# liortalker/MindTheEdge

Hardware: AMD Instinct MI355X
Metric: training images/sec, PackNet-SAN+edge-loss 384x1280 bf16 (higher is better)
Workload: dtype bf16; 1 GPU; T8: PackNet-SAN + silog + 4-scale depth-edge loss training step, 384x1280, 8 frames/GPU, dropout 0.5, flip 0.5; global_batch=8, height=384, width=1280, parallelism=single GPU

## Files before the change

include/mte_kernels.h:

```cpp
#ifndef MTE_KERNELS_H
#define MTE_KERNELS_H

#ifdef __cplusplus
extern "C" {
#endif

typedef struct ihipStream_t* mte_stream_t;

#define MTE_OK 0
#define MTE_ERR_ARG (-1)
#define MTE_ERR_LAUNCH (-2)
#define MTE_ERR_UNSUPPORTED (-3)
#define MTE_DT_BF16 0
#define MTE_DT_F32 1

#define MTE_CONV_ACCUMULATE 1
#define MTE_CONV_SOLO 2
int mte_conv2d_igemm(const void* x, long ldx, const void* wpack, const float* bias, void* y, long ldy, int out_f32,
                     int B, int H, int W, int Cin_p, int N, int KH, int KW, int dtype,
                     float* workspace, long workspace_elems, int accumulate, mte_stream_t stream);
int mte_conv2d_igemm_unshuffle(const void* x, long ldx, const void* wpack, void* y, long ldy,
                               int B, int H, int W, int Cin_p, int N, int KH, int KW, int dtype, int accumulate, mte_stream_t stream);
#define MTE_OPT_GN_PREZEROED 0
#define MTE_OPT_LOSS_PREZEROED 1
// ... 49 lines not shown
                   int B, int HW, int C, float eps, int dtype, mte_stream_t stream);
int mte_gn_tail_fwd(const void* y1, long ld1, const double* stats1, const float* gamma1, const float* beta1,
                    const void* y2, long ld2, const float* scale2, void* t, long ldt, double* stats_t,
                    const float* gamma_t, const float* beta_t, void* z, long ldz,
                    int B, int HW, int C, float eps, int dtype, mte_stream_t stream);

int mte_pack3d_fwd(const void* x, long ldx, const float* w3, const float* b3, void* out, long ldo,
                   int B, int H, int W, int C, int dtype, mte_stream_t stream);
int mte_pack3d_bwd_data(const void* dout, long ldo, const float* w3, void* dx, long lddx,
                        int B, int H, int W, int C, int dtype, mte_stream_t stream);
int mte_pack3d_bwd_weight(const void* x, long ldx, const void* dout, long ldo, float* dwb,
                          int B, int H, int W, int C, int dtype, mte_stream_t stream);
int mte_unpack3d_fwd(const void* x, long ldx, const float* w3, const float* b3, void* out, long ldo,
                     int B, int H, int W, int C, int dtype, mte_stream_t stream);
int mte_unpack3d_bwd_data(const void* dout, long ldo, const float* w3, void* dx, long lddx,
                          int B, int H, int W, int C, int dtype, mte_stream_t stream);
int mte_unpack3d_bwd_weight(const void* x, long ldx, const void* dout, long ldo, float* dwb,
                            int B, int H, int W, int C, int dtype, mte_stream_t stream);

int mte_fold_pack_weights(const float* W, const float* K3, const float* b, const float* b3, float* Wf, float* bf,
                          int Co, int D, int k, mte_stream_t stream);
int mte_unfold_pack_wgrad(const float* dWf, const float* dbf, const float* W, const float* K3, const float* b3,
                          float* dW, float* dk3b, int Co, int D, int k, int accumulate, mte_stream_t stream);
int mte_pixel_shuffle(const void* src, long lds_, void* dst, long ldd, int B, int H, int W, int C, int dir, int dtype, mte_stream_t stream);
int mte_copy_rect(const void* src, long lds_, int Hs, int Ws, int sy, int sx, void* dst, long ldd, int Hd, int Wd, int dy, int dx,
                  int B, int h, int w, int C, int mode, int dtype, mte_stream_t stream);
typedef struct { const void* src; long lds_; int Hs, Ws, sy, sx; void* dst; long ldd; int Hd, Wd, dy, dx, h, w, mode; } mte_rect_op;
int mte_copy_rects(const void* ops, int n, int B, int C, int dtype, mte_stream_t stream);

int mte_invdepth_fwd(const void* x, long ldx, const float* w, const float* bias, float* out,
                     int B, int H, int W, int C, float min_depth, int dtype, mte_stream_t stream);
int mte_invdepth_bwd_data(const float* w, const float* inv_out, const float* dout, float* dlogit,
                          void* dx, long lddx, int B, int H, int W, int C, float min_depth, int dtype, mte_stream_t stream);
long mte_invdepth_bwd_weight_workspace_elems(int C);
int mte_invdepth_bwd_weight(const void* x, long ldx, const float* dlogit, float* dwb, float* records,
                            int B, int H, int W, int C, int dtype, mte_stream_t stream);

int mte_rank1_conv_fwd(const float* inv, const float* w, long w_stride, void* y, long ldy, int B, int h, int wl, int N, int dtype, mte_stream_t stream);
int mte_rank1_conv_bwd_data(const void* dy, long lddy, const float* w, long w_stride, float* dinv, int B, int h, int wl, int N, int accumulate, int dtype,
                            mte_stream_t stream);
int mte_upsample2_f32(const float* inv, float* out, int B, int h, int wl, mte_stream_t stream);
int mte_conv2d_patch_fwd_rank1_ok(const float* bias, long ldx, int B, int H, int W, int Cin_p, int N);
int mte_conv2d_patch_fwd_rank1(const void* x, long ldx, const void* wpatch, const float* bias, void* y, long ldy, int B, int H, int W, int Cin_p, int N,
                               const float* inv, const float* w1, long w1_stride, mte_stream_t stream);
int mte_conv2d_patch_fwd_plus1x1(const void* x, long ldx, const void* wpatch, const float* bias, void* y, long ldy, int B, int H, int W, int Cin_p, int N,
                                 const void* x2, long ldx2, const void* wpatch2, int C2, mte_stream_t stream);
long mte_rank1_conv_bwd_records_elems(int N);
int mte_rank1_conv_bwd_weight(const void* dy, long lddy, const float* inv, float* dw, long dw_stride, float* records,
                              int B, int h, int wl, int N, int dtype, mte_stream_t stream);
int mte_nchw_to_nhwc(const float* src, void* dst, long ldd, int B, int C, int H, int W, int Cp, int flip_w, int dtype, mte_stream_t stream);
int mte_upsample_inv_fwd(const float* inv, void* dst, long ldd, int B, int h, int w, int dtype, mte_stream_t stream);
int mte_upsample_inv_bwd(const void* dsrc, long lds_, float* dinv, int B, int h, int w, int accumulate, int dtype, mte_stream_t stream);
int mte_copy_channels(const void* src, long lds_, void* dst, long ldd, long npix, int C, int dtype, mte_stream_t stream);
int mte_split_record(const float* src, float* dst0, int n0, float* dst1, int n1, mte_stream_t stream);
int mte_add_channels(const void* a, long lda, const void* b, long ldb, void* out, long ldo, long npix, int C, int dtype, mte_stream_t stream);

typedef struct { const float* pred; const float* edge; const float* normal; const float* mask; float* gmap; float* dpred; int H; int W; } mte_edge_scale;
long mte_edge_loss_work_elems(const void* scales, int nscales, int B);
int mte_edge_loss_multi_fwd(const void* scales, int nscales, int B, int from_inv, int is_grad, int is_sigmoid, float thresh,
                            float weight, float pos_to_neg, const float* gt_depth, double* work, float* losses, float* coef,
                            float* silog_loss, float* silog_aux, mte_stream_t stream);
int mte_edge_loss_multi_bwd(const void* scales, int nscales, int B, int from_inv, int is_grad, int is_sigmoid, float thresh,
                            const float* coef, const float* gout, const float* gt_depth, const float* silog_aux, const float* silog_gout,
                            mte_stream_t stream);
long mte_edge_loss_sums_elems(int B, int H, int W);
int mte_edge_loss_fwd(const float* pred, const float* edge, const float* normal, const float* mask, double* sums, float* gmap,
                      int B, int H, int W, int from_inv, int is_grad, int is_sigmoid, float thresh, mte_stream_t stream);
int mte_edge_loss_finalize(const double* sums, int B, long numel, float weight, float pos_to_neg, int has_mask,
                           float out_scale, float* loss_acc, float* loss_this, float* coef, mte_stream_t stream);
int mte_edge_loss_bwd(const float* pred, const float* edge, const float* normal, const float* mask, const float* coef, const float* gout,
                      float* dpred, int B, int H, int W, int from_inv, int is_grad, int is_sigmoid, float thresh, mte_stream_t stream);

long mte_edge_loss_kind_work_elems(int B, int H, int W);
// ... 105 lines not shown
```

mindtheedge_amd/csrc/heads_misc.hip:

```cpp
#include "common.hpp"
#include <atomic>

int tap_wgrad_mfma_launch(const bf16_t* x, long ldx, const float* m, float* rec, long rec_stride, int B, int H, int W, int C, int sgn, int up2, int has_db,
                          int max_wgs, int* groups, hipStream_t st);
namespace {

template <typename T> __device__ __forceinline__ void ld8(const T* p, float* v);
template <> __device__ __forceinline__ void ld8<bf16_t>(const bf16_t* p, float* v) { unpack16<bf16_t>(*(const u32x4_t*)p, v); }
template <> __device__ __forceinline__ void ld8<float>(const float* p, float* v) {
    unpack16<float>(*(const u32x4_t*)p, v); unpack16<float>(*(const u32x4_t*)(p + 4), v + 4);
}
template <typename T> __device__ __forceinline__ void st8(T* p, const float* v);
template <> __device__ __forceinline__ void st8<bf16_t>(bf16_t* p, const float* v) { *(u32x4_t*)p = pack16<bf16_t>(v); }
template <> __device__ __forceinline__ void st8<float>(float* p, const float* v) {
    *(u32x4_t*)p = pack16<float>(v); *(u32x4_t*)(p + 4) = pack16<float>(v + 4);
}

struct HeadArgs {
    const void* x; long ldx;
    const float* w; const float* bias;
    float* out;
    const float* dlogit;
    void* dx; long lddx;
    float* dw;
// ... 153 lines not shown
            for (int s = 0; s < CS; ++s) in[kx][s] = nxt[kx][s];
        if constexpr (PF) { if (r < y1) load_row(r + 1); }
        f32x4_t d = {0.f, 0.f, 0.f, 0.f};
#pragma unroll
        for (int kx = 0; kx < 3; ++kx)
#pragma unroll
            for (int s = 0; s < CS; ++s) {
                d = __builtin_amdgcn_mfma_f32_16x16x32_bf16(__builtin_bit_cast(bf16x8_t, wh[kx][s]), __builtin_bit_cast(bf16x8_t, in[kx][s]), d, 0, 0, 0);
                d = __builtin_amdgcn_mfma_f32_16x16x32_bf16(__builtin_bit_cast(bf16x8_t, wl[kx][s]), __builtin_bit_cast(bf16x8_t, in[kx][s]), d, 0, 0, 0);
            }
        const float done = o_prev + d[2];
        if (kb == 0 && r - 1 >= y0 && r - 1 < y1 && x < a.W) out[(long)(r - 1) * a.W + x] = a.inv_min_depth / (1.f + __expf(-(done + bias)));
        o_prev = o_cur + d[1];
        o_cur = d[0];
    }
}

__global__ void invdepth_dlogit_kernel(const float* __restrict__ dout, const float* __restrict__ inv, float* __restrict__ dl, long n, float s) {
    for (long i = blockIdx.x * (long)blockDim.x + threadIdx.x; i < n; i += (long)gridDim.x * blockDim.x) {
        const float v = inv[i];
        dl[i] = dout[i] * v * (1.f - v / s);
    }
}

struct DlRow { float v[3]; bool ok; };
#define HEAD_LOAD_DL(Y, D)                                                                        \
    {                                                                                             \
        (D).ok = (unsigned)(Y) < (unsigned)a.H;                                                   \
        const long row_ = (long)min(max((Y), 0), a.H - 1) * a.W;                                  \
        _Pragma("unroll") for (int cx = 0; cx < 3; ++cx) (D).v[cx] = dl[row_ + xc[cx]];           \
    }
#define HEAD_DL(D, CX) (((D).ok && xok[CX]) ? (D).v[CX] : 0.f)

template <typename T>
__global__ __launch_bounds__(256) void invdepth_bwd_data_kernel(HeadArgs a) {
    HEAD_MAP();
    float wr[9][8];
#pragma unroll
    for (int t = 0; t < 9; ++t)
#pragma unroll
        for (int i = 0; i < 8; ++i) wr[t][i] = a.w[(c0 + i) * 9 + t];
#pragma unroll 1
    for (int strip = s_first; strip < s_last; ++strip) {
        HEAD_STRIP();
        const float* dl = a.dlogit + (long)b * a.H * a.W;
        T* dx = (T*)a.dx + (long)b * a.H * a.W * a.lddx + c0;
        DlRow d[4];
        HEAD_LOAD_DL(y0 - 1, d[0]) HEAD_LOAD_DL(y0, d[1]) HEAD_LOAD_DL(y0 + 1, d[2])
#define HEAD_BD_STEP(K, R0, R1, R2, R3)                                                           \
    {                                                                                             \
        const int yy = y + K;                                                                     \
        HEAD_LOAD_DL(yy + 2, d[R3])                                                               \
        float dxv[8];                                                                             \
        _Pragma("unroll") for (int i = 0; i < 8; ++i) dxv[i] = 0.f;                               \
        _Pragma("unroll") for (int ty = 0; ty < 3; ++ty)                                          \
            _Pragma("unroll") for (int tx = 0; tx < 3; ++tx) {                                    \
                const float g = ty == 0 ? HEAD_DL(d[R2], 2 - tx) : (ty == 1 ? HEAD_DL(d[R1], 2 - tx) : HEAD_DL(d[R0], 2 - tx)); \
                _Pragma("unroll") for (int i = 0; i < 8; ++i) dxv[i] = fmaf(g, wr[ty * 3 + tx][i], dxv[i]); \
            }                                                                                     \
        if (xin && yy < y1) st8<T>(dx + ((long)yy * a.W + x) * a.lddx, dxv);                      \
    }
        for (int y = y0; y < y1; y += 4) {
            HEAD_BD_STEP(0, 0, 1, 2, 3) HEAD_BD_STEP(1, 1, 2, 3, 0) HEAD_BD_STEP(2, 2, 3, 0, 1) HEAD_BD_STEP(3, 3, 0, 1, 2)
        }
#undef HEAD_BD_STEP
    }
}

template <typename T>
__global__ __launch_bounds__(256) void invdepth_bwd_weight_kernel(HeadArgs a) {
    extern __shared__ float sdw[];
    for (int i = threadIdx.x; i < a.C * 9 + 1; i += 256) sdw[i] = 0.f;
    __syncthreads();
    HEAD_MAP();
    float gw[9][8];
#pragma unroll
    for (int t = 0; t < 9; ++t)
#pragma unroll
        for (int i = 0; i < 8; ++i) gw[t][i] = 0.f;
    float gb = 0.f;
#pragma unroll 1
    for (int strip = s_first; strip < s_last; ++strip) {
        HEAD_STRIP();
        const float* dl = a.dlogit + (long)b * a.H * a.W;
        const T* img = (const T*)a.x + (long)b * a.H * a.W * a.ldx + c0;
        DlRow d[5];
        Ch8<T> xr[4];
        bool xrok[4];
#define HEAD_LOAD_X(Y, S) { xrok[S] = xin && (Y) < y1; xr[S].load(img + ((long)min((Y), a.H - 1) * a.W + xc[1]) * a.ldx); }
        HEAD_LOAD_DL(y0 - 1, d[0]) HEAD_LOAD_DL(y0, d[1]) HEAD_LOAD_DL(y0 + 1, d[2]) HEAD_LOAD_DL(y0 + 2, d[3])
        HEAD_LOAD_X(y0, 0) HEAD_LOAD_X(y0 + 1, 1) HEAD_LOAD_X(y0 + 2, 2)
#define HEAD_BW_STEP(K, R0, R1, R2, R4, X0, X3)                                                   \
// ... 185 lines not shown
                const bool kk = ok && Yok[r];
                win[r][k] = u32x4_t{kk ? v[0] : 0u, kk ? v[1] : 0u, kk ? v[2] : 0u, kk ? v[3] : 0u};
            }
        };
#pragma unroll
        for (int k = 0; k < 4; ++k) load_col(2 * x0 - 1 + k, k);
        const int x1 = min(x0 + SEG, wl);
        for (int x = x0; x < x1; ++x) {
            float acc = 0.f;
            const int woff = cc * P;
#pragma unroll
            for (int r = 0; r < 4; ++r)
#pragma unroll
                for (int k = 0; k < 4; ++k) {
                    float g[P];
                    unpack16<T>(win[r][k], g);
                    const float* wr = wc + (r * 4 + k) * N + woff;
#pragma unroll
                    for (int e = 0; e < P; ++e) acc = fmaf(g[e], wr[e], acc);
                }
            for (int off = 1; off < cpr; off <<= 1) acc += __shfl_xor(acc, off, 64);
            const long pq = ((long)b * h + yl) * wl + x;
            if (live && cc == 0) dinv[pq] = accumulate ? dinv[pq] + acc : acc;
            if (x + 1 < x1) {
#pragma unroll
                for (int r = 0; r < 4; ++r) { win[r][0] = win[r][2]; win[r][1] = win[r][3]; }
                load_col(2 * x + 3, 2);
                load_col(2 * x + 4, 3);
            }
        }
    }
}

template <typename T>
__global__ __launch_bounds__(256) void rank1_conv_bwd_weight_kernel(const T* __restrict__ dy, long lddy, const float* __restrict__ inv, float* __restrict__ records,
                                                                    int B, int h, int wl, int N) {
    extern __shared__ __attribute__((aligned(16))) float sred[];
    constexpr int P = Elem<T>::PER16, SEG = 16;
    const int cpr = N / P, W = 2 * wl, nseg = (wl + SEG - 1) / SEG;
    const long items = (long)B * h * nseg * cpr;
    float dacc[9][P];
#pragma unroll
    for (int tp = 0; tp < 9; ++tp)
#pragma unroll
        for (int e = 0; e < P; ++e) dacc[tp][e] = 0.f;
    const int cc = threadIdx.x % cpr;
    for (long it = blockIdx.x * (long)blockDim.x + threadIdx.x; it < items; it += (long)gridDim.x * blockDim.x) {
        long t = it / cpr;
        const int x0 = (int)(t % nseg) * SEG; t /= nseg;
        const int yl = (int)(t % h); const int b = (int)(t / h);
        const T* base = dy + (((long)b * 2 * h + 2 * yl) * W) * lddy + cc * P;
        const float* ir[3]; bool iok[3];
#pragma unroll
        for (int r = 0; r < 3; ++r) { const int yy = yl - 1 + r; iok[r] = (unsigned)yy < (unsigned)h; ir[r] = inv + ((long)b * h + min(max(yy, 0), h - 1)) * wl; }
        float uw[3][3];
#pragma unroll
        for (int k = 0; k < 3; ++k) {
            const int xx = x0 - 1 + k; const bool ok = (unsigned)xx < (unsigned)wl; const int xc = min(max(xx, 0), wl - 1);
#pragma unroll
            for (int r = 0; r < 3; ++r) uw[r][k] = (ok && iok[r]) ? ir[r][xc] : 0.f;
        }
        const int x1 = min(x0 + SEG, wl);
        for (int x = x0; x < x1; ++x) {
            u32x4_t raw[4];
#pragma unroll
            for (int q = 0; q < 4; ++q) raw[q] = *(const u32x4_t*)(base + ((long)(q >> 1) * W + 2 * x + (q & 1)) * lddy);
// ... 136 lines not shown
    float src = scale * ((float)dst + 0.5f) - 0.5f;
    if (src < 0.f) src = 0.f;
    i0 = (int)src; if (i0 > in - 1) i0 = in - 1;
    i1 = i0 < in - 1 ? i0 + 1 : i0;
    l1 = src - (float)i0;
}
__global__ void resize_bilinear_kernel(const float* __restrict__ x, float* __restrict__ y, float* __restrict__ dx, const float* __restrict__ dy,
                                       int B, int h, int w, int H, int W) {
    const float sh = (float)h / (float)H, sw = (float)w / (float)W;
    const long n = (long)B * H * W;
    for (long i = blockIdx.x * (long)blockDim.x + threadIdx.x; i < n; i += (long)gridDim.x * blockDim.x) {
        const int X = (int)(i % W), Y = (int)((i / W) % H), b = (int)(i / ((long)W * H));
        int y0, y1, x0, x1; float ly, lx;
        bilin_src(Y, h, sh, y0, y1, ly); bilin_src(X, w, sw, x0, x1, lx);
        const long base = (long)b * h * w;
        const float w00 = (1.f - ly) * (1.f - lx), w01 = (1.f - ly) * lx, w10 = ly * (1.f - lx), w11 = ly * lx;
        if (y) {
            y[i] = w00 * x[base + (long)y0 * w + x0] + w01 * x[base + (long)y0 * w + x1] + w10 * x[base + (long)y1 * w + x0] + w11 * x[base + (long)y1 * w + x1];
        } else {
            const float g = dy[i];
            atomicAdd(dx + base + (long)y0 * w + x0, w00 * g); atomicAdd(dx + base + (long)y0 * w + x1, w01 * g);
            atomicAdd(dx + base + (long)y1 * w + x0, w10 * g); atomicAdd(dx + base + (long)y1 * w + x1, w11 * g);
        }
    }
}

inline int stream_grid(long n, int per = 256) { long g = (n + per - 1) / per; return (int)(g > 8192 ? 8192 : (g < 1 ? 1 : g)); }
int g_head_mfma = 1;
inline bool head_ok(int C) { const int cb = C >> 3; return C % 8 == 0 && cb >= 1 && cb <= 64 && (cb & (cb - 1)) == 0; }
inline long head_strips(int B, int H, int W, int C) {
    const int pxw = 256 / (C >> 3);
    return (long)((W + pxw - 1) / pxw) * ((H + HEAD_ROWS - 1) / HEAD_ROWS) * B;
}
template <typename F> int head_resident(F f, size_t lds, std::atomic<int>* cache) {
    int v = cache->load(std::memory_order_relaxed);
    if (v == 0) {
        int per_cu = 0, dev = 0, cus = 256;
        if (hipOccupancyMaxActiveBlocksPerMultiprocessor(&per_cu, f, 256, lds) != hipSuccess || per_cu < 1) per_cu = 2;
        hipDeviceProp_t prop;
        if (hipGetDevice(&dev) == hipSuccess && hipGetDeviceProperties(&prop, dev) == hipSuccess && prop.multiProcessorCount > 0) cus = prop.multiProcessorCount;
        v = per_cu * cus;
        cache->store(v, std::memory_order_relaxed);
    }
    return v;
}
inline long head_record_stride(int C) { return ((long)C * 9 + 1 + 3) / 4 * 4; }
constexpr int HEAD_WGRAD_MAX_BLOCKS = 1024;

}

#ifdef MTE_DEV
extern "C" int mtei_set_head_mfma(int v) { g_head_mfma = v; return MTE_OK; }
#endif

extern "C" {

int mte_invdepth_fwd(const void* x, long ldx, const float* w, const float* bias, float* out,
                     int B, int H, int W, int C, float min_depth, int dtype, hipStream_t stream) {
    (void)hipGetLastError();
    if (!x || !w || !bias || !out || !head_ok(C)) return MTE_ERR_ARG;
    HeadArgs a{}; a.x = x; a.ldx = ldx; a.w = w; a.bias = bias; a.out = out; a.B = B; a.H = H; a.W = W; a.C = C;
    a.inv_min_depth = 1.f / min_depth; a.npix = (long)B * H * W;
    if (dtype == MTE_DT_BF16 && g_head_mfma && C % 32 == 0 && C <= ((g_head_mfma & 2) ? 256 : 128) && ldx % 8 == 0) {
        int rows = C >= 128 ? 16 : 32;
        bool pf = C >= 64;
        if (g_head_mfma != 1) {
            pf = (g_head_mfma & 4) != 0;
            if (g_head_mfma >> 8) rows = g_head_mfma >> 8;
        }
        const long g2 = (long)((W + 63) / 64) * ((H + rows - 1) / rows) * B;
        if (g2 <= 0x7fffffffL) {
#define MTE_HEAD_LAUNCH(CS_)                                                                                                              \
            if (pf) hipLaunchKernelGGL((invdepth_fwd_mfma_kernel<CS_, true>), dim3((unsigned)g2), dim3(256), 0, stream, a, rows);       \
            else hipLaunchKernelGGL((invdepth_fwd_mfma_kernel<CS_, false>), dim3((unsigned)g2), dim3(256), 0, stream, a, rows);         \
            return mte_check_launch();
            switch (C / 32) {
                case 1: { MTE_HEAD_LAUNCH(1) }
                case 2: { MTE_HEAD_LAUNCH(2) }
                case 4: { MTE_HEAD_LAUNCH(4) }
                case 8: { MTE_HEAD_LAUNCH(8) }
            }
#undef MTE_HEAD_LAUNCH
        }
    }
    const long grid = head_strips(B, H, W, C);
    if (grid > 0x7fffffffL) return MTE_ERR_UNSUPPORTED;
    if (dtype == MTE_DT_BF16) hipLaunchKernelGGL(invdepth_fwd_kernel<bf16_t>, dim3((unsigned)grid), dim3(256), 0, stream, a);
    else hipLaunchKernelGGL(invdepth_fwd_kernel<float>, dim3((unsigned)grid), dim3(256), 0, stream, a);
    return mte_check_launch();
}

int mte_invdepth_bwd_data(const float* w, const float* inv_out, const float* dout, float* dlogit,
                          void* dx, long lddx, int B, int H, int W, int C, float min_depth, int dtype, hipStream_t stream) {
    (void)hipGetLastError();
    if (!w || !inv_out || !dout || !dlogit || !dx || !head_ok(C)) return MTE_ERR_ARG;
    const long npix = (long)B * H * W;
    hipLaunchKernelGGL(invdepth_dlogit_kernel, dim3(stream_grid(npix)), dim3(256), 0, stream, dout, inv_out, dlogit, npix, 1.f / min_depth);
    HeadArgs a{}; a.w = w; a.dlogit = dlogit; a.dx = dx; a.lddx = lddx; a.B = B; a.H = H; a.W = W; a.C = C; a.npix = npix;
    const long grid = head_strips(B, H, W, C);
    if (grid > 0x7fffffffL) return MTE_ERR_UNSUPPORTED;
    if (dtype == MTE_DT_BF16) hipLaunchKernelGGL(invdepth_bwd_data_kernel<bf16_t>, dim3((unsigned)grid), dim3(256), 0, stream, a);
    else hipLaunchKernelGGL(invdepth_bwd_data_kernel<float>, dim3((unsigned)grid), dim3(256), 0, stream, a);
    return mte_check_launch();
}

long mte_invdepth_bwd_weight_workspace_elems(int C) { return head_ok(C) ? HEAD_WGRAD_MAX_BLOCKS * head_record_stride(C) : 0; }

int mte_invdepth_bwd_weight(const void* x, long ldx, const float* dlogit, float* dwb, float* records,
                            int B, int H, int W, int C, int dtype, hipStream_t stream) {
    (void)hipGetLastError();
    if (!x || !dlogit || !dwb || !records || !head_ok(C)) return MTE_ERR_ARG;
    const long npix = (long)B * H * W;
    HeadArgs a{}; a.x = x; a.ldx = ldx; a.dlogit = dlogit; a.dw = records; a.rec_stride = head_record_stride(C);
    a.B = B; a.H = H; a.W = W; a.C = C; a.npix = npix;
    const int n = C * 9 + 1;
    if (dtype == MTE_DT_BF16) {
        int groups = 0;
        const int rc = tap_wgrad_mfma_launch((const bf16_t*)x, ldx, dlogit, records, a.rec_stride, B, H, W, C, -1, 0, 1, HEAD_WGRAD_MAX_BLOCKS, &groups, stream);
        if (rc == MTE_OK) {
            hipLaunchKernelGGL(invdepth_reduce_kernel, dim3((n + 63) / 64), dim3(1024), 0, stream, records, a.rec_stride, groups, n, dwb);
            return mte_check_launch();
        }
        if (rc != MTE_ERR_UNSUPPORTED) return rc;
    }
    const size_t lds = sizeof(float) * (C * 9 + 4);
    long g = head_strips(B, H, W, C);
    static std::atomic<int> res_b[64], res_f[64];
    const int ci = (C >> 3) & 63;
    const long res = dtype == MTE_DT_BF16 ? head_resident(invdepth_bwd_weight_kernel<bf16_t>, lds, &res_b[ci]) : head_resident(invdepth_bwd_weight_kernel<float>, lds, &res_f[ci]);
    if (g > res) g = res;
    if (g > HEAD_WGRAD_MAX_BLOCKS) g = HEAD_WGRAD_MAX_BLOCKS;
    if (dtype == MTE_DT_BF16) hipLaunchKernelGGL(invdepth_bwd_weight_kernel<bf16_t>, dim3((unsigned)g), dim3(256), lds, stream, a);
    else hipLaunchKernelGGL(invdepth_bwd_weight_kernel<float>, dim3((unsigned)g), dim3(256), lds, stream, a);
    hipLaunchKernelGGL(invdepth_reduce_kernel, dim3((n + 63) / 64), dim3(1024), 0, stream, records, a.rec_stride, (int)g, n, dwb);
    return mte_check_launch();
}
// ... 14 lines not shown
    if (dtype == MTE_DT_BF16) hipLaunchKernelGGL(upsample_inv_kernel<bf16_t>, dim3(grid), dim3(256), 0, stream, inv, (bf16_t*)dst, ldd, B, h, w);
    else hipLaunchKernelGGL(upsample_inv_kernel<float>, dim3(grid), dim3(256), 0, stream, inv, (float*)dst, ldd, B, h, w);
    return mte_check_launch();
}
int mte_upsample_inv_bwd(const void* dsrc, long lds_, float* dinv, int B, int h, int w, int accumulate, int dtype, hipStream_t stream) {
    (void)hipGetLastError();
    if (!dsrc || !dinv) return MTE_ERR_ARG;
    const int grid = stream_grid((long)B * h * w);
    if (dtype == MTE_DT_BF16) hipLaunchKernelGGL(upsample_inv_bwd_kernel<bf16_t>, dim3(grid), dim3(256), 0, stream, (const bf16_t*)dsrc, lds_, dinv, B, h, w, accumulate);
    else hipLaunchKernelGGL(upsample_inv_bwd_kernel<float>, dim3(grid), dim3(256), 0, stream, (const float*)dsrc, lds_, dinv, B, h, w, accumulate);
    return mte_check_launch();
}

int mte_rank1_conv_fwd(const float* inv, const float* w, long w_stride, void* y, long ldy, int B, int h, int wl, int N, int dtype, hipStream_t stream) {
    (void)hipGetLastError();
    if (!inv || !w || !y || N % 32 != 0 || N > 256 || B < 1 || h < 1 || wl < 1) return MTE_ERR_ARG;
    const int per16 = dtype == MTE_DT_BF16 ? 8 : 4;
    const int grid = stream_grid((long)B * 2 * h * ((2 * wl + 63) / 64) * (N / per16));
    if (dtype == MTE_DT_BF16) hipLaunchKernelGGL(rank1_conv_fwd_kernel<bf16_t>, dim3(grid), dim3(256), 0, stream, inv, w, w_stride, (bf16_t*)y, ldy, B, h, wl, N);
    else hipLaunchKernelGGL(rank1_conv_fwd_kernel<float>, dim3(grid), dim3(256), 0, stream, inv, w, w_stride, (float*)y, ldy, B, h, wl, N);
    return mte_check_launch();
}
int mte_rank1_conv_bwd_data(const void* dy, long lddy, const float* w, long w_stride, float* dinv, int B, int h, int wl, int N, int accumulate, int dtype,
                            hipStream_t stream) {
    (void)hipGetLastError();
    if (!dy || !w || !dinv || (N != 32 && N != 64 && N != 128) || B < 1 || h < 1 || wl < 1) return MTE_ERR_ARG;
    const int per16 = dtype == MTE_DT_BF16 ? 8 : 4;
    const int grid = stream_grid((long)B * h * ((wl + 15) / 16) * (N / per16));
    const size_t lds = sizeof(float) * 25 * N;
    if (dtype == MTE_DT_BF16) hipLaunchKernelGGL(rank1_conv_bwd_data_kernel<bf16_t>, dim3(grid), dim3(256), lds, stream, (const bf16_t*)dy, lddy, w, w_stride, dinv, B, h, wl, N, accumulate);
    else hipLaunchKernelGGL(rank1_conv_bwd_data_kernel<float>, dim3(grid), dim3(256), lds, stream, (const float*)dy, lddy, w, w_stride, dinv, B, h, wl, N, accumulate);
    return mte_check_launch();
}
constexpr int RANK1_BWD_WGS = 1024;
long mte_rank1_conv_bwd_records_elems(int N) { return (long)RANK1_BWD_WGS * N * 9; }
int mte_rank1_conv_bwd_weight(const void* dy, long lddy, const float* inv, float* dw, long dw_stride, float* records,
                              int B, int h, int wl, int N, int dtype, hipStream_t stream) {
    (void)hipGetLastError();
    if (!dy || !inv || !dw || !records || (N != 32 && N != 64 && N != 128) || B < 1 || h < 1 || wl < 1) return MTE_ERR_ARG;
    if (dtype == MTE_DT_BF16) {
        int groups = 0;
        const int rc = tap_wgrad_mfma_launch((const bf16_t*)dy, lddy, inv, records, (long)N * 9, B, 2 * h, 2 * wl, N, +1, 1, 0, RANK1_BWD_WGS, &groups, stream);
        if (rc == MTE_OK) {
            hipLaunchKernelGGL(rank1_wgrad_reduce_kernel, dim3((N * 9 + 3) / 4), dim3(256), 0, stream, records, groups, N, dw, dw_stride);
            return mte_check_launch();
        }
        if (rc != MTE_ERR_UNSUPPORTED) return rc;
    }
    const int per16 = dtype == MTE_DT_BF16 ? 8 : 4;
    const long items = (long)B * h * ((wl + 15) / 16) * (N / per16);
    long g = (items + 255) / 256; if (g > RANK1_BWD_WGS) g = RANK1_BWD_WGS; if (g < 1) g = 1;
    const size_t lds = sizeof(float) * 4 * N * 9;
    if (dtype == MTE_DT_BF16) hipLaunchKernelGGL(rank1_conv_bwd_weight_kernel<bf16_t>, dim3((unsigned)g), dim3(256), lds, stream, (const bf16_t*)dy, lddy, inv, records, B, h, wl, N);
    else hipLaunchKernelGGL(rank1_conv_bwd_weight_kernel<float>, dim3((unsigned)g), dim3(256), lds, stream, (const float*)dy, lddy, inv, records, B, h, wl, N);
    hipLaunchKernelGGL(rank1_wgrad_reduce_kernel, dim3((N * 9 + 3) / 4), dim3(256), 0, stream, records, (int)g, N, dw, dw_stride);
    return mte_check_launch();
}
int mte_upsample2_f32(const float* inv, float* out, int B, int h, int wl, hipStream_t stream) {
    (void)hipGetLastError();
    if (!inv || !out || B < 1 || h < 1 || wl < 1) return MTE_ERR_ARG;
    hipLaunchKernelGGL(upsample2_f32_kernel, dim3(stream_grid((long)B * 4 * h * wl)), dim3(256), 0, stream, inv, out, B, h, wl);
    return mte_check_launch();
}

int mte_copy_channels(const void* src, long lds_, void* dst, long ldd, long npix, int C, int dtype, hipStream_t stream) {
    (void)hipGetLastError();
// ... 61 lines not shown
```

mindtheedge_amd/kernels.py:

```python
import ctypes
import itertools
import math
import os
import weakref

import torch

from ._lib import lib, MteError

DT_BF16, DT_F32 = 0, 1
_state = {"compute_dtype": torch.bfloat16, "weights_epoch": 0}


def set_compute_dtype(dtype):
    dtype = {"bf16": torch.bfloat16, "fp32": torch.float32, "f32": torch.float32}.get(dtype, dtype)
    assert dtype in (torch.bfloat16, torch.float32)
    _state["compute_dtype"] = dtype


def compute_dtype():
    return _state["compute_dtype"]


def bump_weights_epoch():
# ... 870 lines not shown
        yp, ldy = _pl(y)
        w1 = w.detach().data_ptr() + 4 * cm * 9
        xp, ldx = _pl(x)
        if (_cfg["fuse_inv_term"] and pack is not None and _patch_ok(W, Cp, cout, kh, kw, x.dtype)
                and lib.mte_conv2d_patch_fwd_rank1_ok(_ptr(b), ldx, B, H, W, Cp, cout) == 1):
            lib.mte_conv2d_patch_fwd_rank1(xp, ldx, pack.get_patch(wm, 'f').data_ptr(), _ptr(b), yp, ldy, B, H, W, Cp, cout,
                                           invc.data_ptr(), w1, cin * 9, _stream())
        else:
            lib.mte_rank1_conv_fwd(invc.data_ptr(), w1, cin * 9, yp, ldy, B, H // 2, W // 2, cout, _dt(y), _stream())
            conv_forward(x, wf, b, cout, kh, kw, out=y, pack=pack, w=wm, accumulate=True)
        z, stats = _gn_forward(y, None, None, gamma, beta, GN_EPS, out=None if out is None else alias_of(out))
        ctx.save_for_backward(x, invc, w, wm, y, stats, gamma, beta)
        ctx.pack = pack
        ctx.bias = b
        return z

    @staticmethod
    def backward(ctx, dz):
        x, invc, w, wm, y, stats, gamma, beta = ctx.saved_tensors
        b = ctx.bias
        cout, cin, kh, kw = w.shape
        cm = cin - 1
        B, Cp, H, W = x.shape
        gg, sg = _grad_dst(gamma, zero=True)
        gb, sb = _grad_dst(beta, zero=True)
        gbias, sbias = _grad_dst(b, zero=True)
        gw, sw = _grad_dst(w)
        dy, _, dgamma, dbeta, db = _gn_backward(dz, y, None, None, stats, gamma, beta, GN_EPS, False, want_dbias=True,
                                                dgamma=gg, dbeta=gb, dbias=gbias)
        dyp, lddy = _pl(dy)

        dinv = torch.empty((B, 1, H // 2, W // 2), dtype=torch.float32, device=x.device)
        wl = w.detach()
        lib.mte_rank1_conv_bwd_data(dyp, lddy, wl.data_ptr() + 4 * cm * 9, cin * 9, dinv.data_ptr(), B, H // 2, W // 2, cout, 0, _dt(dy), _stream())

        def weight_gradients():
            dwm, _ = _conv_wgrad(x, dy, wm, False, None, None)
            gw[:, :cm].copy_(dwm)
            rec = torch.empty((int(lib.mte_rank1_conv_bwd_records_elems(cout)),), dtype=torch.float32, device=x.device)
            lib.mte_rank1_conv_bwd_weight(dyp, lddy, invc.data_ptr(), gw.data_ptr() + 4 * cm * 9, cin * 9, rec.data_ptr(), B, H // 2, W // 2, cout, _dt(dy), _stream())

        if sw and _side["enabled"]:
            if _side["keep_bytes"] > _SIDE_KEEP_LIMIT:
                join_side_stream()
            with torch.cuda.stream(_side_stream_for(x, dy, invc)):
                weight_gradients()
        else:
            weight_gradients()
        dx = None
        if ctx.needs_input_grad[0]:
            dx = conv_backward(x, dy, wm, ctx.pack, True, need_dw=False, need_dbias=False, fork_slot=ctx.fork_slot)[0]
        if not ctx.needs_input_grad[1]:
            dinv = None
        return dx, dinv, _grad_ret(w, gw, sw), _grad_ret(b, db, sbias), _grad_ret(gamma, dgamma, sg), _grad_ret(beta, dbeta, sb), None, None


class ConvFn(torch.autograd.Function):

    @staticmethod
    def forward(ctx, x, w, b, pack, bias_grad=True):
        ctx.fork_slot = getattr(x, "_mte_fork_slot", None)
        wf, _ = pack.get(w, x.dtype, bool(ctx.needs_input_grad[0]))
        cout, cin, kh, kw = w.shape
        y = conv_forward(x, wf, b, cout, kh, kw, pack=pack, w=w)
        ctx.save_for_backward(x, w)
        ctx.pack = pack
        ctx.bias = b
# ... 448 lines not shown
            else:
                g3, gb3 = _deliver_pair(w3, b3, dk3b, 108)
            return (g3, gb3, _grad_ret(w, dw_band, gw_sunk), _grad_ret(b, db, gb_sunk))

        if _side["enabled"] and _all_sunk(w3, b3, w, b):
            with torch.cuda.stream(_side_stream_for(P, dy, T1, T2, dyb1, dyb2, dTs[0], dTs[1], xb1, xb2, Wf)):
                g3, gb3, gw, gb = weight_grads()
        else:
            g3, gb3, gw, gb = weight_grads()
        dx = new_act(B, C, H, W, P.dtype, dev)
        if not _dgrad_unshuffled(dy, Wf, pack_fold, dx, k + 2):
            dP, _, _ = conv_backward(P, dy, Wf, pack_fold, True, need_dw=False)
            sp, lds_ = _pl(dP)
            dp_, ldd = _pl(dx)
            lib.mte_pixel_shuffle(sp, lds_, dp_, ldd, B, H, W, C, 1, dt, _stream())
        bands.join()
        _rects([(dxb[0][:B], 0, 0, dx, 0, 0, 2 * hb, W, 1), (dxb[0][B:], 0, 0, dx, H - 2 * hb, 0, 2 * hb, W, 1)])
        _rects([(dxb[1][:B], 0, 0, dx, 0, 0, H, 2 * hb, 1), (dxb[1][B:], 0, 0, dx, 0, W - 2 * hb, H, 2 * hb, 1)])
        return (dx, g3, gb3, gw, gb, _grad_ret(gamma, dgamma, sg), _grad_ret(beta, dbeta, sbt), None, None, None)


class InvDepthFn(torch.autograd.Function):

    @staticmethod
    def forward(ctx, x, w, b, min_depth):
        B, C, H, W = x.shape
        out = torch.empty((B, 1, H, W), dtype=torch.float32, device=x.device)
        xp, ldx = _pl(x)
        wc = w.detach().contiguous().float()
        lib.mte_invdepth_fwd(xp, ldx, wc.data_ptr(), b.detach().float().data_ptr(), out.data_ptr(), B, H, W, C, min_depth, _dt(x), _stream())
        ctx.save_for_backward(x, wc, out)
        ctx.min_depth = min_depth
        ctx.params = (w, b)
        return out

    @staticmethod
    def backward(ctx, dout):
        x, wc, out = ctx.saved_tensors
        w, b = ctx.params
        B, C, H, W = x.shape
        dout = dout.contiguous().float()
        dx = new_act(B, C, H, W, x.dtype, x.device)
        dlogit = torch.empty((B, H, W), dtype=torch.float32, device=x.device)
        dxp, lddx = _pl(dx)
        lib.mte_invdepth_bwd_data(wc.data_ptr(), out.data_ptr(), dout.data_ptr(), dlogit.data_ptr(), dxp, lddx,
                                  B, H, W, C, ctx.min_depth, _dt(x), _stream())

        def weight_grads():
            xp, ldx = _pl(x)
            dst = _claim_adjacent(w, b) if tuple(w.shape) == (1, C, 3, 3) and b.numel() == 1 else None
            dwb = dst if dst is not None else torch.empty((C * 9 + 1,), dtype=torch.float32, device=x.device)
            rec = torch.empty((int(lib.mte_invdepth_bwd_weight_workspace_elems(C)),), dtype=torch.float32, device=x.device)
            lib.mte_invdepth_bwd_weight(xp, ldx, dlogit.data_ptr(), dwb.data_ptr(), rec.data_ptr(), B, H, W, C, _dt(x), _stream())
            if dst is not None:
                _announce(w, b)
                return None, None
            return _deliver_pair(w, b, dwb, C * 9)

        if _side["enabled"] and _all_sunk(w, b):
            with torch.cuda.stream(_side_stream_for(x, dlogit)):
                dw, db = weight_grads()
        else:
            dw, db = weight_grads()
        return dx, dw, db, None


def _pending_slot(slot):
    while slot is not None:
        if slot["buf"] is not None:
            return slot if "pending" in slot else None
        slot = slot["parent"]
    return None


def _flush_pending(slot):
    dy3, w3, pack3 = slot.pop("pending")
    dx = slot["buf"]
    B, Cp, H, W = dx.shape
    cout = w3.shape[0]
# ... 134 lines not shown
```

Baseline: 380.4 images/sec.

## Accumulate invdepth dx into fork-slot buffer and add row-strip rank1 bwd-data kernel

The inverse-depth head backward can now add its input gradient directly into a pre-existing fork-slot gradient buffer through a new accumulate variant of the kernel. This avoids allocating a separate dx and summing the branch gradients later. The rank-1 conv backward-data path switches to a new 512-thread kernel. That kernel folds the 3x3 weights into per-phase sums, walks row strips sized to the resident block count, and reduces across channels with LDS plus shuffles. The cost is more complex indexing, extra loads of the existing dx in the accumulate path, and a dependency on fork-slot bookkeeping being correct.

```diff
diff --git a/include/mte_kernels.h b/include/mte_kernels.h
--- a/include/mte_kernels.h
+++ b/include/mte_kernels.h
@@ -105,6 +105,8 @@
                      int B, int H, int W, int C, float min_depth, int dtype, mte_stream_t stream);
 int mte_invdepth_bwd_data(const float* w, const float* inv_out, const float* dout, float* dlogit,
                           void* dx, long lddx, int B, int H, int W, int C, float min_depth, int dtype, mte_stream_t stream);
+int mte_invdepth_bwd_data_acc(const float* w, const float* inv_out, const float* dout, float* dlogit,
+                              void* dx, long lddx, int B, int H, int W, int C, float min_depth, int dtype, mte_stream_t stream);
 long mte_invdepth_bwd_weight_workspace_elems(int C);
 int mte_invdepth_bwd_weight(const void* x, long ldx, const float* dlogit, float* dwb, float* records,
                             int B, int H, int W, int C, int dtype, mte_stream_t stream);
@@ -112,6 +114,8 @@
 int mte_rank1_conv_fwd(const float* inv, const float* w, long w_stride, void* y, long ldy, int B, int h, int wl, int N, int dtype, mte_stream_t stream);
 int mte_rank1_conv_bwd_data(const void* dy, long lddy, const float* w, long w_stride, float* dinv, int B, int h, int wl, int N, int accumulate, int dtype,
                             mte_stream_t stream);
+int mte_rank1_conv_bwd_data_rows(const void* dy, long lddy, const float* w, long w_stride, float* dinv, int B, int h, int wl, int N, int accumulate, int dtype,
+                                 mte_stream_t stream);
 int mte_upsample2_f32(const float* inv, float* out, int B, int h, int wl, mte_stream_t stream);
 int mte_conv2d_patch_fwd_rank1_ok(const float* bias, long ldx, int B, int H, int W, int Cin_p, int N);
 int mte_conv2d_patch_fwd_rank1(const void* x, long ldx, const void* wpatch, const float* bias, void* y, long ldy, int B, int H, int W, int Cin_p, int N,
diff --git a/mindtheedge_amd/csrc/heads_misc.hip b/mindtheedge_amd/csrc/heads_misc.hip
--- a/mindtheedge_amd/csrc/heads_misc.hip
+++ b/mindtheedge_amd/csrc/heads_misc.hip
@@ -209,7 +209,7 @@
     }
 #define HEAD_DL(D, CX) (((D).ok && xok[CX]) ? (D).v[CX] : 0.f)
 
-template <typename T>
+template <typename T, bool ACC>
 __global__ __launch_bounds__(256) void invdepth_bwd_data_kernel(HeadArgs a) {
     HEAD_MAP();
     float wr[9][8];
@@ -224,10 +224,17 @@
         T* dx = (T*)a.dx + (long)b * a.H * a.W * a.lddx + c0;
         DlRow d[4];
         HEAD_LOAD_DL(y0 - 1, d[0]) HEAD_LOAD_DL(y0, d[1]) HEAD_LOAD_DL(y0 + 1, d[2])
+        Ch8<T> on[4];
+        if constexpr (ACC) {
+#pragma unroll
+            for (int k = 0; k < 4; ++k) on[k].load(dx + ((long)min(y0 + k, y1 - 1) * a.W + xc[1]) * a.lddx);
+        }
 #define HEAD_BD_STEP(K, R0, R1, R2, R3)                                                           \
     {                                                                                             \
         const int yy = y + K;                                                                     \
         HEAD_LOAD_DL(yy + 2, d[R3])                                                               \
+        Ch8<T> oc;                                                                                \
+        if constexpr (ACC) { oc = on[K]; on[K].load(dx + ((long)min(yy + 4, y1 - 1) * a.W + xc[1]) * a.lddx); } \
         float dxv[8];                                                                             \
         _Pragma("unroll") for (int i = 0; i < 8; ++i) dxv[i] = 0.f;                               \
         _Pragma("unroll") for (int ty = 0; ty < 3; ++ty)                                          \
@@ -235,6 +242,11 @@
                 const float g = ty == 0 ? HEAD_DL(d[R2], 2 - tx) : (ty == 1 ? HEAD_DL(d[R1], 2 - tx) : HEAD_DL(d[R0], 2 - tx)); \
                 _Pragma("unroll") for (int i = 0; i < 8; ++i) dxv[i] = fmaf(g, wr[ty * 3 + tx][i], dxv[i]); \
             }                                                                                     \
+        if constexpr (ACC) {                                                                      \
+            float ov[8];                                                                          \
+            oc.get(ov);                                                                           \
+            _Pragma("unroll") for (int i = 0; i < 8; ++i) dxv[i] = ov[i] + dxv[i];                \
+        }                                                                                         \
         if (xin && yy < y1) st8<T>(dx + ((long)yy * a.W + x) * a.lddx, dxv);                      \
     }
         for (int y = y0; y < y1; y += 4) {
@@ -486,6 +498,89 @@
     }
 }
 
+constexpr int RANK1_ROWS_NT = 512, RANK1_ROWS_MIN = 8;
+template <typename T>
+__global__ __launch_bounds__(RANK1_ROWS_NT) void rank1_conv_bwd_data_rows_kernel(const T* __restrict__ dy, long lddy, const float* __restrict__ w, long wstride,
+                                                                                 float* __restrict__ dinv, int B, int h, int wl, int N, int accumulate, int rows) {
+    extern __shared__ __attribute__((aligned(16))) float sw[];
+    float* wc = sw + 9 * N;
+    float* sx = wc + 16 * N;
+    for (int i = threadIdx.x; i < 9 * N; i += blockDim.x) sw[i] = w[(long)(i % N) * wstride + i / N];
+    __syncthreads();
+    for (int i = threadIdx.x; i < 16 * N; i += blockDim.x) {
+        const int c = i % N, r = i / N, ry = r >> 2, rx = r & 3;
+        float s = 0.f;
+        for (int qy = 0; qy < 2; ++qy)
+            for (int qx = 0; qx < 2; ++qx) {
+                const int ky = qy + 2 - ry, kx = qx + 2 - rx;
+                if ((unsigned)ky < 3u && (unsigned)kx < 3u) s += sw[(ky * 3 + kx) * N + c];
+            }
+        wc[i] = s;
+    }
+    __syncthreads();
+    constexpr int P = Elem<T>::PER16, NT = RANK1_ROWS_NT;
+    const int cpr = N / P, cw = NT / cpr, ow = cw / 2 - 1;
+    const int cc = threadIdx.x % cpr, c = threadIdx.x / cpr;
+    const int H = 2 * h, W = 2 * wl;
+    const int tiles = (wl + ow - 1) / ow, strips = (h + rows - 1) / rows;
+    int id = blockIdx.x;
+    const int xb = (id % tiles) * ow; id /= tiles;
+    const int y0 = (id % strips) * rows, y1 = min(h, y0 + rows); const int b = id / strips;
+    const int X = 2 * xb - 1 + c;
+    const bool Xok = (unsigned)X < (unsigned)W;
+    float wa[4][P], wn[4][P];
+#pragma unroll
+    for (int r = 0; r < 4; ++r)
+#pragma unroll
+        for (int e = 0; e < P; ++e) {
+            wa[r][e] = wc[(r * 4 + (c & 1)) * N + cc * P + e];
+            wn[r][e] = wc[(r * 4 + 2 + (c & 1)) * N + cc * P + e];
+        }
+    const T* base = dy + ((long)b * H * W + min(max(X, 0), W - 1)) * lddy + cc * P;
+    struct Pair { u32x4_t v0, v1; };
+    auto load_pair = [&](int p) __attribute__((always_inline)) {
+        Pair q;
+        q.v0 = *(const u32x4_t*)(base + (long)max(2 * p - 1, 0) * W * lddy);
+        q.v1 = *(const u32x4_t*)(base + (long)min(2 * p, H - 1) * W * lddy);
+        return q;
+    };
+    Pair q0 = load_pair(y0), q1 = load_pair(min(y0 + 1, y1)), q2;
+    float ca = 0.f, cn = 0.f;
+    const bool finisher = cc == 0 && (c & 1) == 0 && (c >> 1) < ow && xb + (c >> 1) < wl;
+    for (int p = y0; p <= y1; ++p) {
+        q2 = load_pair(min(p + 2, y1));
+        float g0[P], g1[P];
+        {
+            const bool k0 = Xok && p >= 1, k1 = Xok && p < h;
+            const u32x4_t z0 = u32x4_t{k0 ? q0.v0[0] : 0u, k0 ? q0.v0[1] : 0u, k0 ? q0.v0[2] : 0u, k0 ? q0.v0[3] : 0u};
+            const u32x4_t z1 = u32x4_t{k1 ? q0.v1[0] : 0u, k1 ? q0.v1[1] : 0u, k1 ? q0.v1[2] : 0u, k1 ? q0.v1[3] : 0u};
+            unpack16<T>(z0, g0); unpack16<T>(z1, g1);
+        }
+        float fa = ca, fn = cn;
+        ca = 0.f; cn = 0.f;
+#pragma unroll
+        for (int e = 0; e < P; ++e) { ca = fmaf(g0[e], wa[0][e], ca); cn = fmaf(g0[e], wn[0][e], cn); }
+#pragma unroll
+        for (int e = 0; e < P; ++e) { ca = fmaf(g1[e], wa[1][e], ca); cn = fmaf(g1[e], wn[1][e], cn); }
+#pragma unroll
+        for (int e = 0; e < P; ++e) { fa = fmaf(g0[e], wa[2][e], fa); fn = fmaf(g0[e], wn[2][e], fn); }
+#pragma unroll
+        for (int e = 0; e < P; ++e) { fa = fmaf(g1[e], wa[3][e], fa); fn = fmaf(g1[e], wn[3][e], fn); }
+        if (p > y0) {
+            float* slot = sx + ((p & 1) ? NT : 0);
+            slot[threadIdx.x] = fn;
+            __syncthreads();
+            float t = fa + (c + 2 < cw ? slot[threadIdx.x + 2 * cpr] : 0.f);
+            for (int off = 1; off < 2 * cpr; off <<= 1) t += __shfl_xor(t, off, 64);
+            if (finisher) {
+                const long pq = ((long)b * h + (p - 1)) * wl + xb + (c >> 1);
+                dinv[pq] = accumulate ? dinv[pq] + t : t;
+            }
+        }
+        q0 = q1; q1 = q2;
+    }
+}
+
 template <typename T>
 __global__ __launch_bounds__(256) void rank1_conv_bwd_weight_kernel(const T* __restrict__ dy, long lddy, const float* __restrict__ inv, float* __restrict__ records,
                                                                     int B, int h, int wl, int N) {
@@ -688,11 +783,11 @@
     const int pxw = 256 / (C >> 3);
     return (long)((W + pxw - 1) / pxw) * ((H + HEAD_ROWS - 1) / HEAD_ROWS) * B;
 }
-template <typename F> int head_resident(F f, size_t lds, std::atomic<int>* cache) {
+template <typename F> int head_resident(F f, size_t lds, std::atomic<int>* cache, int threads = 256) {
     int v = cache->load(std::memory_order_relaxed);
     if (v == 0) {
         int per_cu = 0, dev = 0, cus = 256;
-        if (hipOccupancyMaxActiveBlocksPerMultiprocessor(&per_cu, f, 256, lds) != hipSuccess || per_cu < 1) per_cu = 2;
+        if (hipOccupancyMaxActiveBlocksPerMultiprocessor(&per_cu, f, threads, lds) != hipSuccess || per_cu < 1) per_cu = 2;
         hipDeviceProp_t prop;
         if (hipGetDevice(&dev) == hipSuccess && hipGetDeviceProperties(&prop, dev) == hipSuccess && prop.multiProcessorCount > 0) cus = prop.multiProcessorCount;
         v = per_cu * cus;
@@ -746,8 +841,8 @@
     return mte_check_launch();
 }
 
-int mte_invdepth_bwd_data(const float* w, const float* inv_out, const float* dout, float* dlogit,
-                          void* dx, long lddx, int B, int H, int W, int C, float min_depth, int dtype, hipStream_t stream) {
+static int invdepth_bwd_data_launch(const float* w, const float* inv_out, const float* dout, float* dlogit,
+                                    void* dx, long lddx, int B, int H, int W, int C, float min_depth, int dtype, bool acc, hipStream_t stream) {
     (void)hipGetLastError();
     if (!w || !inv_out || !dout || !dlogit || !dx || !head_ok(C)) return MTE_ERR_ARG;
     const long npix = (long)B * H * W;
@@ -755,9 +850,22 @@
     HeadArgs a{}; a.w = w; a.dlogit = dlogit; a.dx = dx; a.lddx = lddx; a.B = B; a.H = H; a.W = W; a.C = C; a.npix = npix;
     const long grid = head_strips(B, H, W, C);
     if (grid > 0x7fffffffL) return MTE_ERR_UNSUPPORTED;
-    if (dtype == MTE_DT_BF16) hipLaunchKernelGGL(invdepth_bwd_data_kernel<bf16_t>, dim3((unsigned)grid), dim3(256), 0, stream, a);
-    else hipLaunchKernelGGL(invdepth_bwd_data_kernel<float>, dim3((unsigned)grid), dim3(256), 0, stream, a);
-    return mte_check_launch();
+    if (dtype == MTE_DT_BF16) {
+        if (acc) hipLaunchKernelGGL((invdepth_bwd_data_kernel<bf16_t, true>), dim3((unsigned)grid), dim3(256), 0, stream, a);
+        else hipLaunchKernelGGL((invdepth_bwd_data_kernel<bf16_t, false>), dim3((unsigned)grid), dim3(256), 0, stream, a);
+    } else {
+        if (acc) hipLaunchKernelGGL((invdepth_bwd_data_kernel<float, true>), dim3((unsigned)grid), dim3(256), 0, stream, a);
+        else hipLaunchKernelGGL((invdepth_bwd_data_kernel<float, false>), dim3((unsigned)grid), dim3(256), 0, stream, a);
+    }
+    return mte_check_launch();
+}
+int mte_invdepth_bwd_data(const float* w, const float* inv_out, const float* dout, float* dlogit,
+                          void* dx, long lddx, int B, int H, int W, int C, float min_depth, int dtype, hipStream_t stream) {
+    return invdepth_bwd_data_launch(w, inv_out, dout, dlogit, dx, lddx, B, H, W, C, min_depth, dtype, false, stream);
+}
+int mte_invdepth_bwd_data_acc(const float* w, const float* inv_out, const float* dout, float* dlogit,
+                              void* dx, long lddx, int B, int H, int W, int C, float min_depth, int dtype, hipStream_t stream) {
+    return invdepth_bwd_data_launch(w, inv_out, dout, dlogit, dx, lddx, B, H, W, C, min_depth, dtype, true, stream);
 }
 
 long mte_invdepth_bwd_weight_workspace_elems(int C) { return head_ok(C) ? HEAD_WGRAD_MAX_BLOCKS * head_record_stride(C) : 0; }
@@ -838,6 +946,27 @@
     else hipLaunchKernelGGL(rank1_conv_bwd_data_kernel<float>, dim3(grid), dim3(256), lds, stream, (const float*)dy, lddy, w, w_stride, dinv, B, h, wl, N, accumulate);
     return mte_check_launch();
 }
+int mte_rank1_conv_bwd_data_rows(const void* dy, long lddy, const float* w, long w_stride, float* dinv, int B, int h, int wl, int N, int accumulate, int dtype,
+                                 hipStream_t stream) {
+    (void)hipGetLastError();
+    if (!dy || !w || !dinv || (N != 32 && N != 64 && N != 128) || B < 1 || h < 1 || wl < 1) return MTE_ERR_ARG;
+    const int per16 = dtype == MTE_DT_BF16 ? 8 : 4;
+    const int ow = RANK1_ROWS_NT / (N / per16) / 2 - 1;
+    const long cols = (long)((wl + ow - 1) / ow) * B;
+    const size_t lds = sizeof(float) * (25 * N + 2 * RANK1_ROWS_NT);
+    static std::atomic<int> res_b[3], res_f[3];
+    const int ci = N == 32 ? 0 : (N == 64 ? 1 : 2);
+    const long res = dtype == MTE_DT_BF16 ? head_resident(rank1_conv_bwd_data_rows_kernel<bf16_t>, lds, &res_b[ci], RANK1_ROWS_NT)
+                                          : head_resident(rank1_conv_bwd_data_rows_kernel<float>, lds, &res_f[ci], RANK1_ROWS_NT);
+    const long strips = res / cols;
+    int rows = strips > 0 ? (int)((h + strips - 1) / strips) : h;
+    if (rows < RANK1_ROWS_MIN) rows = RANK1_ROWS_MIN;
+    const long grid = cols * ((h + rows - 1) / rows);
+    if (grid > 0x7fffffffL) return MTE_ERR_UNSUPPORTED;
+    if (dtype == MTE_DT_BF16) hipLaunchKernelGGL(rank1_conv_bwd_data_rows_kernel<bf16_t>, dim3((unsigned)grid), dim3(RANK1_ROWS_NT), lds, stream, (const bf16_t*)dy, lddy, w, w_stride, dinv, B, h, wl, N, accumulate, rows);
+    else hipLaunchKernelGGL(rank1_conv_bwd_data_rows_kernel<float>, dim3((unsigned)grid), dim3(RANK1_ROWS_NT), lds, stream, (const float*)dy, lddy, w, w_stride, dinv, B, h, wl, N, accumulate, rows);
+    return mte_check_launch();
+}
 constexpr int RANK1_BWD_WGS = 1024;
 long mte_rank1_conv_bwd_records_elems(int N) { return (long)RANK1_BWD_WGS * N * 9; }
 int mte_rank1_conv_bwd_weight(const void* dy, long lddy, const float* inv, float* dw, long dw_stride, float* records,
diff --git a/mindtheedge_amd/kernels.py b/mindtheedge_amd/kernels.py
--- a/mindtheedge_amd/kernels.py
+++ b/mindtheedge_amd/kernels.py
@@ -926,7 +926,7 @@
 
         dinv = torch.empty((B, 1, H // 2, W // 2), dtype=torch.float32, device=x.device)
         wl = w.detach()
-        lib.mte_rank1_conv_bwd_data(dyp, lddy, wl.data_ptr() + 4 * cm * 9, cin * 9, dinv.data_ptr(), B, H // 2, W // 2, cout, 0, _dt(dy), _stream())
+        lib.mte_rank1_conv_bwd_data_rows(dyp, lddy, wl.data_ptr() + 4 * cm * 9, cin * 9, dinv.data_ptr(), B, H // 2, W // 2, cout, 0, _dt(dy), _stream())
 
         def weight_gradients():
             dwm, _ = _conv_wgrad(x, dy, wm, False, None, None)
@@ -1441,6 +1441,7 @@
         ctx.save_for_backward(x, wc, out)
         ctx.min_depth = min_depth
         ctx.params = (w, b)
+        ctx.fork_slot = getattr(x, "_mte_fork_slot", None)
         return out
 
     @staticmethod
@@ -1449,11 +1450,15 @@
         w, b = ctx.params
         B, C, H, W = x.shape
         dout = dout.contiguous().float()
-        dx = new_act(B, C, H, W, x.dtype, x.device)
         dlogit = torch.empty((B, H, W), dtype=torch.float32, device=x.device)
+        slot = ctx.fork_slot
+        target = _fork_target(slot, (B, C, H, W), x.dtype)
+        dx = target if target is not None else new_act(B, C, H, W, x.dtype, x.device)
         dxp, lddx = _pl(dx)
-        lib.mte_invdepth_bwd_data(wc.data_ptr(), out.data_ptr(), dout.data_ptr(), dlogit.data_ptr(), dxp, lddx,
-                                  B, H, W, C, ctx.min_depth, _dt(x), _stream())
+        bwd_data = lib.mte_invdepth_bwd_data_acc if target is not None else lib.mte_invdepth_bwd_data
+        bwd_data(wc.data_ptr(), out.data_ptr(), dout.data_ptr(), dlogit.data_ptr(), dxp, lddx, B, H, W, C, ctx.min_depth, _dt(x), _stream())
+        if slot is not None:
+            slot["buf"] = dx
 
         def weight_grads():
             xp, ldx = _pl(x)
```

After: 382.6 images/sec (median of 6 runs). About the same (+0.6%).
